# Cyan4973/FiniteStateEntropy

Measured on AMD Instinct MI355X. Metric: MB/s encode+decode per GPU on 32KB probagen blocks; bit-exact vs CPU ref, higher is better.
Workload: dtype u8; 1 GPU; probagen Proba14, 100000 x 32KB blocks per GPU, FSE encode+decode (one-shot calls at the reference's default limits: tableLog 11, decode maxLog 12), bit-exact check; blocks_per_gpu=100000, block_bytes=32768, codec=fse, parity=fse: roundtrip-all-blocks

## Files before the change

### finitestateentropy_amd/csrc/fse_tables.hip

```cpp
#include "internal.h"

#include "wave_glue.h"
#include "ncount_reader.h"
#include "fse_wave_build.h"

DEV void fse_wave_build_ctable(const WaveBuildLds& w, const int nn[4], u32 maxSV, u32 tl, u32* img, u32 lane)
{
    u16* const cumAll = w.cumP;
    *(uint2*)(w.nrm + 4 * lane) = make_uint2(((u32)nn[0] & 0xFFFFu) | ((u32)nn[1] << 16), ((u32)nn[2] & 0xFFFFu) | ((u32)nn[3] << 16));
    __syncthreads();
    const u32 ts = 1u << tl;
    u16* const stateTable = (u16*)(img + 1);
    u32* const tt = img + 1 + (ts >> 1);
    {
        u32 eff[4], laneSum = 0;
#pragma unroll
        for (int i = 0; i < 4; ++i) { eff[i] = nn[i] == -1 ? 1u : (u32)nn[i]; laneSum += eff[i]; }
        u32 total;
        u32 run = wb_scan_excl(laneSum, lane, &total);
#pragma unroll
        for (int i = 0; i < 4; ++i) {
            const u32 s = 4 * lane + i;
            cumAll[s] = (u16)run;
            if (s <= maxSV) {
                if (nn[i] == 0) { tt[2 * s] = 0; tt[2 * s + 1] = ((tl + 1) << 16) - ts; }
                else if (nn[i] == -1 || nn[i] == 1) { tt[2 * s] = run - 1u; tt[2 * s + 1] = (tl << 16) - ts; }
                else {
                    const u32 maxBitsOut = tl - hibit32((u32)nn[i] - 1);
                    tt[2 * s] = run - (u32)nn[i];
                    tt[2 * s + 1] = (maxBitsOut << 16) - ((u32)nn[i] << maxBitsOut);
                }
            }
            run += eff[i];
        }
        if (lane == 0) img[0] = tl | (maxSV << 16);
    }
    __syncthreads();
    wave_spread_rank(w, maxSV, tl, lane, [&](u32 s) { return (u32)cumAll[s]; },
                     [&](u32 u, u32 s, u32 r, u32 first) { (void)s; stateTable[first + r] = (u16)(ts + u); });
}

__global__ __launch_bounds__(64) void k_fse_cprep(FseCPrepArgs a, u32 capTs)
{
    extern __shared__ __attribute__((aligned(16))) u8 wbLds[];
    const size_t b = blockIdx.x;
    const u32 lane = threadIdx.x;
    const size_t n = view_size(a.src, b);
    FseMeta m; m.state = 0; m.hdrSize = 0; m.tableLog = 0; m.maxSV = 0; m.pace = 0;
    const size_t top = a.histResults[b];
    size_t result = 0; bool go = false;
    if (n <= 1) result = 0;
    else if (is_err(top)) result = top;
    else if (top == n) result = 1;
    else if (top == 1 || top < (n >> 7)) result = 0;
    else go = true;
    const WaveBuildLds w = wave_build_carve(wbLds, capTs);
    u32* const hdrImg = w.cnt;
    u32 maxSV = 0, tl = 0;
    int nn[4] = { 0, 0, 0, 0 };
    if (go) {
        maxSV = a.maxSVs[b];
        tl = wg_optimal_tablelog(a.tableLogReq, n, maxSV, 2);
        const uint4 cv = ((const uint4*)(a.counts + b * 256))[lane];
        const u32 c[4] = { cv.x, cv.y, cv.z, cv.w };
        for (u32 i = lane; i < 136; i += 64) hdrImg[i] = 0;
        const size_t e = wg_normalize<64>(nn, c, (u64)n, maxSV, tl, lane);
        if (is_err(e)) { result = e; go = false; }
    }
    __syncthreads();
    if (go) {
        const size_t h = wg_write_ncount<64>(hdrImg, a.dstCapacity, nn, maxSV, tl, lane);
        if (is_err(h)) { result = h; go = false; }
        else m.hdrSize = (u32)h;
    }
    __syncthreads();
    if (!go) { if (lane == 0) { a.meta[b] = m; a.results[b] = result; } return; }
    {   u8* const dst = a.dst + b * a.dstStride;
        const u8* const hb = (const u8*)hdrImg;
        for (u32 i = lane; i < m.hdrSize; i += 64) dst[i] = hb[i];
    }
    int top1 = nn[0] > nn[1] ? nn[0] : nn[1]; top1 = nn[2] > top1 ? nn[2] : top1; top1 = nn[3] > top1 ? nn[3] : top1;
    top1 = wave_max_i32(top1);
    m.state = ((u32)top1 * 64u > (63u << tl) || n < FSE_ENC_WAVE_MIN) ? FSE_ENC_LANE : FSE_ENC_PAR;
    {
        u32 present = (nn[0] != 0) + (nn[1] != 0) + (nn[2] != 0) + (nn[3] != 0);
        present = wg_sum<64>(present);
        const u32 mix = (1u << tl) / (present ? present : 1u);
        m.pace = mix < 64u ? 0u : mix < 128u ? 1u : mix < 256u ? 2u : 3u;
    }
    m.tableLog = tl; m.maxSV = maxSV;
    if (lane == 0) a.meta[b] = m;
    fse_wave_build_ctable(w, nn, maxSV, tl, a.ctables + b * a.ctStrideU32, lane);
}

__global__ __launch_bounds__(64) void k_fse_dparse(FseDPrepArgs a)
{
    const size_t b = (size_t)blockIdx.x * 64 + threadIdx.x;
    const u32 lane = threadIdx.x;
    int cls = -1;
    if (b < a.nBlocks) {
        FseMeta m; m.state = 0; m.hdrSize = 0; m.tableLog = 0; m.maxSV = 0; m.pace = 0; m.pace = 0;
        const u8* const in = view_ptr(a.csrc, b);
        const size_t cSize = view_size(a.csrc, b);
        size_t result = 0;
        bool done = false;
        if (a.rawRle) { const size_t orig = a.origSizes ? a.origSizes[b] : a.uniformOrig; done = cSize == orig || cSize == 1; }
        if (!done) do {
            u32 tl = 0, maxSV = 255;
            s16* const norm = a.norms + b * 256;
            const size_t h = ncount_read<1>(norm, &maxSV, &tl, in, cSize);
            if (is_err(h)) { result = h; break; }
            if (tl > a.maxLog) { result = FERR(tableLog_tooLarge); break; }
            cls = FSE_DCLS_REV11;
            if (tl > FSE_DEC_FAST_MAXLOG) {
                int top = 0;
                for (u32 s = 0; s <= maxSV; ++s) top = norm[s] > top ? norm[s] : top;
                cls = 2 * top > (1 << tl) ? FSE_DCLS_PLAIN : FSE_DCLS_REV12;
            }
            m.state = 1u | ((u32)cls << 2); m.hdrSize = (u32)h; m.tableLog = tl; m.maxSV = maxSV;
        } while (0);
        a.meta[b] = m;
        if (m.state == 0 && !done) a.results[b] = result;
    }
    if (cls >= 0) { const size_t bin = view_size(a.csrc, b) >> FSE_DBIN_LOG; cls = cls * FSE_DBINS + (int)(bin < FSE_DBINS - 1 ? bin : FSE_DBINS - 1); }
    const unsigned long long below = (1ull << lane) - 1ull;
    unsigned long long todo = __ballot(cls >= 0);
    while (todo) {
        const int leader = __builtin_ctzll(todo);
        const int c = __shfl(cls, leader, WAVE);
        const unsigned long long mask = __ballot(cls == c);
        u32 base = 0;
        if ((int)lane == leader) {
            base = atomicAdd(&a.counts[c], (u32)__builtin_popcountll(mask));
            atomicAdd(&a.counts[FSE_DCLS_COUNT + c / FSE_DBINS], (u32)__builtin_popcountll(mask));
        }
        base = (u32)__shfl((int)base, leader, WAVE);
        if (cls == c) a.lists[(size_t)c * a.nBlocks + base + (u32)__builtin_popcountll(mask & below)] = (u32)b;
        todo &= ~mask;
    }
}

__global__ __launch_bounds__(64) void k_fse_dbuild(FseDPrepArgs a, u32 capTs, int firstList, int nLists, u32 ldsCapTs)
{
    extern __shared__ __attribute__((aligned(16))) u8 wbLds[];
    {   u32 total = 0;
        for (int k = firstList / (int)FSE_DBINS; k < (firstList + nLists) / (int)FSE_DBINS; ++k) total += a.counts[FSE_DCLS_COUNT + k];
        if (blockIdx.x >= total) return;
    }
    constexpr int MAXL = 2 * FSE_DBINS;
    static_assert(FSE_DBINS % 4 == 0, "the list lengths are read as 16-byte vectors");
    uint4 cv[MAXL / 4];
#pragma unroll
    for (int i = 0; i < MAXL / 4; ++i) cv[i] = 4 * i < nLists ? ((const uint4*)(a.counts + firstList))[i] : make_uint4(0, 0, 0, 0);
    u32 idx = blockIdx.x;
    int c = firstList + nLists;
    {   u32 before = 0; bool found = false;
#pragma unroll
        for (int i = 0; i < MAXL; ++i) {
            const uint4 v = cv[i >> 2];
            const u32 n = (i & 3) == 0 ? v.x : (i & 3) == 1 ? v.y : (i & 3) == 2 ? v.z : v.w;
            const bool here = !found & (i < nLists) & (idx < before + n);
            c = here ? firstList + i : c; idx = here ? idx - before : idx;
            found |= here;
            before += n;
        }
    }
    if (c == firstList + nLists) return;
    const size_t b = a.lists[(size_t)c * a.nBlocks + idx];
    const u32 lane = threadIdx.x;
    const FseMeta m = a.meta[b];
    if (m.state == 0) return;
    const WaveBuildLds w = wave_build_carve(wbLds, ldsCapTs);
    *(uint2*)(w.nrm + 4 * lane) = *(const uint2*)(a.norms + b * 256 + 4 * lane);
    __syncthreads();
    const u32 tl = m.tableLog, ts = 1u << tl;
    const bool rev = ((m.state >> 2) & 3u) != FSE_DCLS_PLAIN;
    u16* const A = a.atab + b * capTs;
    u8* const S = a.symtab + b * capTs;
    const bool fast = wave_spread_rank(w, m.maxSV, tl, lane, [&](u32 s) { return (u32)(int)w.nrm[s]; }, [&](u32 u, u32 s, u32 r, u32 nrm) {
        const int n = (int)nrm;
        const u32 next = (n > 0 ? (u32)n : 1u) + r;
        const u32 nb = tl - hibit32(next);
        const u32 ns = (next << nb) - ts;
        const u32 x = rev ? __brev(u) >> (32u - tl) : u;
        A[x] = rev ? (u16)(nb | ((__brev(ns) >> (32u - tl)) << 5)) : (u16)((ns & 0xFFFu) | (nb << 12));
        S[x] = (u8)s;
    });
    if (lane == 0) a.meta[b].state = m.state | (fast ? 2u : 0u);
}

__global__ __launch_bounds__(256) void k_fse_export_dtable(FseDPrepArgs a, u32 capTs, u32* dtables, size_t dtStrideU32)
{
    const size_t b = blockIdx.x;
    const FseMeta m = a.meta[b];
    if (m.state == 0) return;
    const u32 tl = m.tableLog, ts = 1u << tl;
    const bool rev = ((m.state >> 2) & 3u) != FSE_DCLS_PLAIN;
    const u16* const A = a.atab + b * capTs;
    const u8* const S = a.symtab + b * capTs;
    u32* const dt = dtables + b * dtStrideU32;
    if (threadIdx.x == 0) dt[0] = tl | ((m.state & 2u) ? 1u << 16 : 0u);
    for (u32 x = threadIdx.x; x < ts; x += blockDim.x) {
        const u32 i = rev ? __brev(x) >> (32u - tl) : x;
        const u32 c = A[i];
        const u32 nb = rev ? (c & 31u) : (c >> 12);
        const u32 ns = rev ? __brev(c >> 5) >> (32u - tl) : (c & 0xFFFu);
        dt[1 + x] = ns | ((u32)S[i] << 16) | (nb << 24);
    }
}
hipError_t launch_fse_export_dtables(const FseDPrepArgs& a, u32* dtables, size_t dtStrideU32, hipStream_t s)
{
    if (a.nBlocks == 0) return hipSuccess;
    hipLaunchKernelGGL(k_fse_export_dtable, dim3((unsigned)a.nBlocks), dim3(256), 0, s, a, 1u << a.maxLog, dtables, dtStrideU32);
    return hipGetLastError();
}

DEV size_t fse_norm_load_checked(int nn[4], const s16* nb, u32 maxSV, u32 tl, u32 maxTl, u32 lane)
{
    if (maxSV > 255u) return FERR(maxSymbolValue_tooLarge);
    if (tl > maxTl) return FERR(tableLog_tooLarge);
    if (tl == 0 || tl == 1 || tl == 3) return FERR(GENERIC);
    u32 cells = 0; bool bad = false;
#pragma unroll
    for (int i = 0; i < 4; ++i) {
        nn[i] = 4 * lane + i <= maxSV ? (int)nb[4 * lane + i] : 0;
        bad |= nn[i] < -1;
        cells += nn[i] == -1 ? 1u : nn[i] > 0 ? (u32)nn[i] : 0u;
    }
    cells = wg_sum<64>(cells);
    return (wg_any<64>(bad, lane) || cells != (1u << tl)) ? FERR(GENERIC) : 0;
}
__global__ __launch_bounds__(64) void k_fse_ctable_from_norm(const s16* norms, size_t normStride, const u32* maxSVs, u32 tl, u32* ctables, size_t ctStrideU32,
                                                            size_t* results, u32 capTs)
{
    extern __shared__ __attribute__((aligned(16))) u8 wbLds[];
    const size_t b = blockIdx.x;
    const u32 lane = threadIdx.x;
    const u32 maxSV = maxSVs[b];
    int nn[4] = { 0, 0, 0, 0 };
    const size_t r = fse_norm_load_checked(nn, norms + b * normStride, maxSV, tl, FSE_MAX_TL, lane);
    if (lane == 0) results[b] = r;
    if (is_err(r)) return;
    fse_wave_build_ctable(wave_build_carve(wbLds, capTs), nn, maxSV, tl, ctables + b * ctStrideU32, lane);
}
hipError_t launch_fse_ctable_from_norm(const s16* norms, size_t normStride, const u32* maxSVs, u32 tl, u32* ctables, size_t ctStrideU32, size_t* results,
                                       size_t nBlocks, hipStream_t s)
{
    if (nBlocks == 0) return hipSuccess;
    const u32 capTs = 1u << (tl >= 1 && tl <= FSE_MAX_TL ? tl : FSE_MAX_TL);
    hipLaunchKernelGGL(k_fse_ctable_from_norm, dim3((unsigned)nBlocks), dim3(64), wave_build_lds_bytes(capTs), s, norms, normStride, maxSVs, tl, ctables, ctStrideU32,
                       results, capTs);
    return hipGetLastError();
}

__global__ __launch_bounds__(64) void k_fse_dmeta_from_norm(FseDPrepArgs a, const s16* norms, size_t normStride, const u32* maxSVs, u32 tl)
{
    const size_t b = blockIdx.x;
    const u32 lane = threadIdx.x;
    const u32 maxSV = maxSVs[b];
    int nn[4] = { 0, 0, 0, 0 };
    const size_t r = fse_norm_load_checked(nn, norms + b * normStride, maxSV, tl, a.maxLog, lane);
    FseMeta m; m.state = 0; m.hdrSize = 0; m.tableLog = tl; m.maxSV = maxSV; m.pace = 0;
    if (!is_err(r)) {
        *(uint2*)(a.norms + b * 256 + 4 * lane) = make_uint2(((u32)nn[0] & 0xFFFFu) | ((u32)nn[1] << 16), ((u32)nn[2] & 0xFFFFu) | ((u32)nn[3] << 16));
        int top = nn[0] > nn[1] ? nn[0] : nn[1]; top = nn[2] > top ? nn[2] : top; top = nn[3] > top ? nn[3] : top;
        top = wave_max_i32(top);
        const u32 cls = tl <= FSE_DEC_FAST_MAXLOG ? (u32)FSE_DCLS_REV11 : 2 * top > (1 << tl) ? (u32)FSE_DCLS_PLAIN : (u32)FSE_DCLS_REV12;
        m.state = 1u | (cls << 2);
        if (lane == 0) {
            const u32 at = atomicAdd(&a.counts[cls * FSE_DBINS], 1u);
            atomicAdd(&a.counts[FSE_DCLS_COUNT + cls], 1u);
            a.lists[(size_t)cls * FSE_DBINS * a.nBlocks + at] = (u32)b;
        }
    }
    if (lane == 0) { a.meta[b] = m; if (is_err(r)) a.results[b] = r; }
}
hipError_t launch_fse_dprep_from_norm(const FseDPrepArgs& a, const s16* norms, size_t normStride, const u32* maxSVs, u32 tl, hipStream_t s)
{
    if (a.nBlocks == 0) return hipSuccess;
    const u32 capTs = 1u << a.maxLog;
    hipError_t e = launch_zero_u32(a.counts, FSE_DCLS_COUNT + FSE_DCLS_KINDS, s);
    if (e != hipSuccess) return e;
    hipLaunchKernelGGL(k_fse_dmeta_from_norm, dim3((unsigned)a.nBlocks), dim3(64), 0, s, a, norms, normStride, maxSVs, tl);
    const u32 capA = a.maxLog < FSE_DEC_FAST_MAXLOG ? capTs : (1u << FSE_DEC_FAST_MAXLOG);
    hipLaunchKernelGGL(k_fse_dbuild, dim3((unsigned)a.nBlocks), dim3(64), wave_build_lds_bytes(capA), s, a, capTs, (int)FSE_DCLS_REV11 * FSE_DBINS, (int)FSE_DBINS, capA);
    if (a.maxLog > FSE_DEC_FAST_MAXLOG)
        hipLaunchKernelGGL(k_fse_dbuild, dim3((unsigned)a.nBlocks), dim3(64), wave_build_lds_bytes(capTs), s, a, capTs, (int)FSE_DCLS_REV12 * FSE_DBINS, 2 * (int)FSE_DBINS, capTs);
    return hipGetLastError();
}

#ifdef FSE_WB_TIMING
extern "C" __attribute__((visibility("default"))) int FSEHIP_debug_wbTiming(unsigned long long* host) { return (int)hipMemcpyFromSymbol(host, HIP_SYMBOL(g_wbTiming), sizeof(g_wbTiming)); }
#endif
__global__ __launch_bounds__(64) void k_fse_glue_normalize(s16* norms, size_t normStride, u32 tlReq, const u32* counts, size_t countStride,
                                                          const size_t* totals, const u32* maxSVs, size_t* results)
{
    const size_t b = blockIdx.x;
    const u32 lane = threadIdx.x;
    const u32 maxSV = maxSVs[b] > 255u ? 255u : maxSVs[b];
    const u32* const cb = counts + b * countStride;
    u32 c[4];
#pragma unroll
    for (int i = 0; i < 4; ++i) c[i] = 4 * lane + i <= maxSV ? cb[4 * lane + i] : 0u;
    int nn[4] = { 0, 0, 0, 0 };
    const u32 tl = tlReq ? tlReq : FSE_DEF_TL;
    const u64 total = (u64)totals[b];
    size_t r = total ? wg_normalize<64>(nn, c, total, maxSV, tl, lane) : FERR(GENERIC);
    if (!is_err(r)) r = tl;
    s16* const nb = norms + b * normStride;
#pragma unroll
    for (int i = 0; i < 4; ++i) if (4 * lane + i <= maxSV && !is_err(r)) nb[4 * lane + i] = (s16)nn[i];
    if (lane == 0) results[b] = r;
}

__global__ __launch_bounds__(64) void k_fse_glue_write_ncount(u8* headers, size_t headerStride, size_t headerCapacity, const s16* norms, size_t normStride,
                                                             const u32* maxSVs, u32 tl, size_t* results)
{
    __shared__ u32 img[136];
    const size_t b = blockIdx.x;
    const u32 lane = threadIdx.x;
    const u32 maxSV = maxSVs[b];
    size_t r;
    if (tl > FSE_MAX_TL) r = FERR(tableLog_tooLarge);
    else if (tl < FSE_MIN_TL || maxSV > 255u) r = FERR(GENERIC);
    else {
        const s16* const nb = norms + b * normStride;
        int nn[4];
#pragma unroll
        for (int i = 0; i < 4; ++i) nn[i] = 4 * lane + i <= maxSV ? (int)nb[4 * lane + i] : 0;
        for (u32 i = lane; i < 136; i += 64) img[i] = 0;
        __syncthreads();
        r = wg_write_ncount<64>(img, headerCapacity, nn, maxSV, tl, lane);
        __syncthreads();
        if (!is_err(r)) {
            u8* const dst = headers + b * headerStride;
            const u8* const hb = (const u8*)img;
            for (u32 i = lane; i < (u32)r; i += 64) dst[i] = hb[i];
        }
    }
    if (lane == 0) results[b] = r;
}

__global__ __launch_bounds__(64) void k_fse_glue_read_ncount(s16* norms, size_t normStride, u32* maxSVs, u32* tableLogs, BlockView headers, size_t nBlocks, size_t* results)
{
    const size_t b = (size_t)blockIdx.x * 64 + threadIdx.x;
    if (b >= nBlocks) return;
    u32 maxSV = maxSVs[b], tl = 0;
    size_t r;
    if ((size_t)maxSV >= normStride) r = FERR(maxSymbolValue_tooLarge);
    else r = ncount_read<1>(norms + b * normStride, &maxSV, &tl, view_ptr(headers, b), view_size(headers, b));
    if (!is_err(r)) { maxSVs[b] = maxSV; tableLogs[b] = tl; }
    results[b] = r;
}

hipError_t launch_fse_glue_normalize(s16* norms, size_t normStride, u32 tl, const u32* counts, size_t countStride, const size_t* totals, const u32* maxSVs,
                                     size_t* results, size_t nBlocks, hipStream_t s)
{
    if (nBlocks == 0) return hipSuccess;
    hipLaunchKernelGGL(k_fse_glue_normalize, dim3((unsigned)nBlocks), dim3(64), 0, s, norms, normStride, tl, counts, countStride, totals, maxSVs, results);
    return hipGetLastError();
}
hipError_t launch_fse_glue_write_ncount(u8* headers, size_t headerStride, size_t headerCapacity, const s16* norms, size_t normStride, const u32* maxSVs, u32 tl,
                                        size_t* results, size_t nBlocks, hipStream_t s)
{
    if (nBlocks == 0) return hipSuccess;
    hipLaunchKernelGGL(k_fse_glue_write_ncount, dim3((unsigned)nBlocks), dim3(64), 0, s, headers, headerStride, headerCapacity, norms, normStride, maxSVs, tl, results);
    return hipGetLastError();
}
hipError_t launch_fse_glue_read_ncount(s16* norms, size_t normStride, u32* maxSVs, u32* tableLogs, const BlockView& headers, size_t* results, size_t nBlocks, hipStream_t s)
{
    if (nBlocks == 0) return hipSuccess;
    hipLaunchKernelGGL(k_fse_glue_read_ncount, dim3((unsigned)((nBlocks + 63) / 64)), dim3(64), 0, s, norms, normStride, maxSVs, tableLogs, headers, nBlocks, results);
    return hipGetLastError();
}

hipError_t launch_fse_cprep(const FseCPrepArgs& a, hipStream_t s)
{
    if (a.nBlocks == 0) return hipSuccess;
    const u32 capTs = 1u << a.maxTl;
    const size_t ldsBytes = wave_build_lds_bytes(capTs);
    probe_before(PK_FSE_CPREP, s);
    hipLaunchKernelGGL(k_fse_cprep, dim3((unsigned)a.nBlocks), dim3(64), ldsBytes, s, a, capTs);
    probe_after(PK_FSE_CPREP, s);
    return hipGetLastError();
}
hipError_t launch_fse_dprep(const FseDPrepArgs& a, hipStream_t s)
{
    if (a.nBlocks == 0) return hipSuccess;
    const u32 capTs = 1u << a.maxLog;
    hipError_t e = launch_zero_u32(a.counts, FSE_DCLS_COUNT + FSE_DCLS_KINDS, s);
    if (e != hipSuccess) return e;
    probe_before(PK_FSE_DPREP, s);
    hipLaunchKernelGGL(k_fse_dparse, dim3((unsigned)((a.nBlocks + 63) / 64)), dim3(64), 0, s, a);
    const u32 capA = a.maxLog < FSE_DEC_FAST_MAXLOG ? capTs : (1u << FSE_DEC_FAST_MAXLOG);
    hipLaunchKernelGGL(k_fse_dbuild, dim3((unsigned)a.nBlocks), dim3(64), wave_build_lds_bytes(capA), s, a, capTs, (int)FSE_DCLS_REV11 * FSE_DBINS, (int)FSE_DBINS, capA);
    if (a.maxLog > FSE_DEC_FAST_MAXLOG)
        hipLaunchKernelGGL(k_fse_dbuild, dim3((unsigned)a.nBlocks), dim3(64), wave_build_lds_bytes(capTs), s, a, capTs, (int)FSE_DCLS_REV12 * FSE_DBINS, 2 * (int)FSE_DBINS, capTs);
    probe_after(PK_FSE_DPREP, s);
    return hipGetLastError();
}
```

### finitestateentropy_amd/csrc/fse_wave_build.h

```cpp
#pragma once
#include "dev_common.h"

#define WB_MAXSYM 256
#ifndef WB_WIN
#define WB_WIN 64u
#endif
#define WB_TSTEP(ts) (((ts) >> 1) + ((ts) >> 3) + 3)

#ifdef FSE_WB_TIMING
__device__ unsigned long long g_wbTiming[4096 * 8];
#define WBT(k) TT[k] = __builtin_readcyclecounter();
#else
#define WBT(k)
#endif
struct WaveBuildLds {
    s16* nrm;
    u16* cumP;
    u8*  symP;
    u8*  symTab;
    u16* marks;
    u32* cnt;
    u16* coarse;
};
__host__ __device__ inline u32 wb_ci(u32 u) { return u + ((u >> 5) << 1); }
__host__ __device__ inline u32 wb_si(u32 u) { return u + ((u >> 5) << 2); }
#ifndef WB_EXTRA_LDS
#define WB_EXTRA_LDS 0u
#endif
__host__ __device__ inline size_t wb_part_a(u32 capTs) { const size_t m = 2 * (size_t)wb_ci(capTs); return m > WB_WIN * 64 ? m : WB_WIN * 64; }
__host__ __device__ inline size_t wb_part_b(u32 capTs) { const size_t t = wb_si(capTs); return t > WB_WIN * 32 ? t : WB_WIN * 32; }
__host__ __device__ inline size_t wave_build_lds_bytes(u32 capTs) { return wb_part_a(capTs) + wb_part_b(capTs) + 512 + 520 + 256 + WB_EXTRA_LDS; }
DEV WaveBuildLds wave_build_carve(u8* base, u32 capTs)
{
    WaveBuildLds w;
    w.cnt = (u32*)base; w.marks = (u16*)base; base += wb_part_a(capTs);
    w.coarse = (u16*)base; w.symTab = base; base += wb_part_b(capTs);
    w.nrm = (s16*)base; base += 512;
    w.cumP = (u16*)base; base += 520;
    w.symP = base;
    return w;
}

DEV u32 wb_bytesum(u32 v) { return __builtin_amdgcn_sad_u8(v, 0u, 0u); }
DEV u32 wb_scan_excl(u32 v, u32 lane, u32* total)
{
#if FSEHIP_DPP_SCANS
    const u32 incl = group_scan_incl<64, ScanAdd>(v, lane);
    *total = group_last<64>(incl, lane);
#else
    u32 incl = v;
#pragma unroll
    for (int off = 1; off < 64; off <<= 1) { const u32 o = (u32)__shfl_up((int)incl, off, WAVE); if ((int)lane >= off) incl += o; }
    *total = (u32)__shfl((int)incl, 63, WAVE);
#endif
    return incl - v;
}

DEV void wb_opaque(u32& v) { asm volatile("" : "+v"(v)); }
#define WB_MAXC ((1u << FSEHIP_FSE_MAX_TABLELOG) >> 6)

template <class Payload, class Emit>
DEV bool wave_spread_rank(const WaveBuildLds& w, u32 maxSV, u32 tl, u32 lane, Payload&& payload, Emit&& emit)
{
#ifdef FSE_WB_TIMING
    unsigned long long TT[8];
#endif
    WBT(0)
    const u32 ts = 1u << tl, mask = ts - 1, step = WB_TSTEP(ts);
    const u32 C = ts >= 64 ? ts >> 6 : 1;
    const bool act = lane * C < ts;
    const u32 m0 = lane * C;
    u16* const marks = w.marks;
    int n[4];
    {   const uint2 raw = *(const uint2*)(w.nrm + 4 * lane);
        n[0] = (s16)(raw.x & 0xFFFFu); n[1] = (s16)(raw.x >> 16); n[2] = (s16)(raw.y & 0xFFFFu); n[3] = (s16)(raw.y >> 16);
    }
    u32 lanePos = 0, laneLow = 0, laneAny = 0; bool big = false;
#pragma unroll
    for (int i = 0; i < 4; ++i) {
        if (4 * lane + i > maxSV) n[i] = 0;
        lanePos += n[i] > 0 ? (u32)n[i] : 0u; laneLow += n[i] == -1; laneAny += n[i] != 0;
        big |= n[i] >= (int)(ts >> 1);
    }
    u32 totals;
    const u32 base3 = wb_scan_excl(lanePos | (laneLow << 13) | (laneAny << 22), lane, &totals);
    u32 posBase = base3 & 0x1FFFu, lowBase = (base3 >> 13) & 0x1FFu, anyBase = base3 >> 22;
    const u32 nLow = (totals >> 13) & 0x1FFu, nAny = totals >> 22;
    const int high = (int)ts - 1 - (int)nLow;
    if (act) { if (C >= 2) for (u32 i = 0; i < C; i += 2) *(u32*)(marks + wb_ci(m0 + i)) = 0; else marks[wb_ci(m0)] = 0; }
    __syncthreads();
    WBT(1)
#pragma unroll
    for (int i = 0; i < 4; ++i) {
        if (n[i] != 0) w.symP[anyBase++] = (u8)(4 * lane + i);
        if (n[i] > 0) { marks[wb_ci(posBase)] = (u16)(4 * lane + i + 1); posBase += (u32)n[i]; }
        else if (n[i] == -1) { w.symTab[wb_si(ts - 1 - lowBase)] = (u8)(4 * lane + i); ++lowBase; }
    }
    u32 nv = 0;
    if (act) { u32 u = (m0 * step) & mask; for (u32 i = 0; i < C; ++i) { nv += (int)u <= high; u = (u + step) & mask; } }
    u32 totalKept;
    const u32 k0 = wb_scan_excl(nv, lane, &totalKept);
    __syncthreads();
    WBT(2)
    u32 localMax = 0;
    for (u32 i = 0; i < nv; i += 8) {
        u32 v[8];
#pragma unroll
        for (u32 j = 0; j < 8; ++j) { const u32 idx = k0 + i + j; v[j] = marks[wb_ci(idx < ts ? idx : ts - 1)]; }
#pragma unroll
        for (u32 j = 0; j < 8; ++j) if (i + j < nv) localMax = v[j] > localMax ? v[j] : localMax;
    }
    u32 run = localMax;
#if FSEHIP_DPP_SCANS
    run = group_scan_incl<64, ScanMax>(run, lane);
    run = dpp_mov<0x138, 0xF, true>(0u, run);
#else
#pragma unroll
    for (int off = 1; off < 64; off <<= 1) { const u32 o = (u32)__shfl_up((int)run, off, WAVE); if ((int)lane >= off) run = o > run ? o : run; }
    run = (u32)__shfl_up((int)run, 1, WAVE);
    if (lane == 0) run = 0;
#endif
    if (act && nv) {
        u32 u = (m0 * step) & mask, k = k0;
        u32 i = 0;
        for (; i + 8 <= C; i += 8) {
            u32 uu[8], v[8]; bool keep[8];
#pragma unroll
            for (u32 j = 0; j < 8; ++j) {
                uu[j] = u; keep[j] = (int)u <= high;
                v[j] = marks[wb_ci(k < ts ? k : ts - 1)];
                k += keep[j]; u = (u + step) & mask;
            }
#pragma unroll
            for (u32 j = 0; j < 8; ++j) if (keep[j]) { run = v[j] > run ? v[j] : run; w.symTab[wb_si(uu[j])] = (u8)(run - 1u); }
        }
        for (; i < C; ++i) {
            if ((int)u <= high) { const u32 v = marks[wb_ci(k)]; ++k; run = v > run ? v : run; w.symTab[wb_si(u)] = (u8)(run - 1u); }
            u = (u + step) & mask;
        }
    }
    __syncthreads();
    WBT(3)

    const u32 nj = C < 8 ? C : 8;
    u32 sym[WB_MAXC / 4], lr[WB_MAXC / 4];
#pragma unroll
    for (u32 q = 0; q < WB_MAXC / 4; ++q) { sym[q] = 0; lr[q] = 0; }
    if (act) {
        if (C >= 8) {
#pragma unroll
            for (u32 g = 0; g < WB_MAXC / 8; ++g)
                if (8 * g < C) {
                    const u32* const syp = (const u32*)(w.symTab + wb_si(m0 + 8 * g));
                    sym[2 * g] = syp[0]; sym[2 * g + 1] = syp[1];
                }
        } else {
#pragma unroll
            for (u32 j = 0; j < 4; ++j) if (j < C) sym[0] |= (u32)w.symTab[wb_si(m0 + j)] << (8 * j);
        }
    }
    const u32 sh8 = 8 * (lane & 3u), grp = lane >> 2;
    const u32 belowMask = (1u << sh8) - 1u;
    const bool single = maxSV < WB_WIN;
    for (u32 base = 0; base <= maxSV; base += WB_WIN) {
        {   const u32 rows = (maxSV + 1 - base) < WB_WIN ? (maxSV + 1 - base) : WB_WIN;
            for (u32 i = 4 * lane; i < rows * 16; i += 256) *(uint4*)(w.cnt + i) = make_uint4(0, 0, 0, 0);
        }
        __syncthreads();
        if (act) {
#pragma unroll
            for (u32 g = 0; g < WB_MAXC / 8; ++g) {
                if (8 * g >= C) break;
                wb_opaque(sym[2 * g]); wb_opaque(sym[2 * g + 1]);
                u32 old[8]; bool in[8];
#pragma unroll
                for (u32 j = 0; j < 8; ++j) {
                    const u32 s = ((sym[2 * g + (j >> 2)] >> (8 * (j & 3))) & 0xFFu) - base;
                    in[j] = j < nj && (single || s < WB_WIN);
                    old[j] = 0;
                    if (in[j]) old[j] = atomicAdd(&w.cnt[s * 16 + grp], 1u << sh8);
                }
#pragma unroll
                for (u32 h = 0; h < 2; ++h) {
                    u32 r = lr[2 * g + h];
#pragma unroll
                    for (u32 k = 0; k < 4; ++k) {
                        const u32 j = 4 * h + k;
                        if (in[j]) r = (r & ~(0xFFu << (8 * k))) | (((old[j] >> sh8) & 0xFFu) << (8 * k));
                    }
                    lr[2 * g + h] = r;
                }
            }
        }
        __syncthreads();
        WBT(4)
        for (u32 j = lane; j < nAny; j += 64) {
            const u32 s = (u32)w.symP[j] - base;
            if (!single && s >= WB_WIN) continue;
            const uint4* const row = (const uint4*)(w.cnt + s * 16);
            const uint4 c0 = row[0], c1 = row[1], c2 = row[2], c3 = row[3];
            u32 r[16];
            u32 acc = 0;
#define WB_ACC(k, v) r[k] = acc; acc += wb_bytesum(v);
            WB_ACC(0, c0.x) WB_ACC(1, c0.y) WB_ACC(2, c0.z) WB_ACC(3, c0.w) WB_ACC(4, c1.x) WB_ACC(5, c1.y) WB_ACC(6, c1.z) WB_ACC(7, c1.w)
            WB_ACC(8, c2.x) WB_ACC(9, c2.y) WB_ACC(10, c2.z) WB_ACC(11, c2.w) WB_ACC(12, c3.x) WB_ACC(13, c3.y) WB_ACC(14, c3.z) WB_ACC(15, c3.w)
#undef WB_ACC
            uint4* const out = (uint4*)(w.coarse + s * 16);
            out[0] = make_uint4(r[0] | (r[1] << 16), r[2] | (r[3] << 16), r[4] | (r[5] << 16), r[6] | (r[7] << 16));
            out[1] = make_uint4(r[8] | (r[9] << 16), r[10] | (r[11] << 16), r[12] | (r[13] << 16), r[14] | (r[15] << 16));
        }
        __syncthreads();
        WBT(5)
        if (act) {
#pragma unroll
            for (u32 g = 0; g < WB_MAXC / 8; ++g) {
                if (8 * g >= C) break;
                wb_opaque(sym[2 * g]); wb_opaque(sym[2 * g + 1]);
                u32 mg = m0 + 8 * g; wb_opaque(mg);
                u32 sf[8], co[8], cn[8], pl[8]; bool in[8];
#pragma unroll
                for (u32 j = 0; j < 8; ++j) {
                    sf[j] = (sym[2 * g + (j >> 2)] >> (8 * (j & 3))) & 0xFFu;
                    const u32 sw = sf[j] - base;
                    in[j] = j < nj && (single || sw < WB_WIN);
                    const u32 row = in[j] ? sw : 0u;
                    co[j] = w.coarse[row * 16 + grp]; cn[j] = w.cnt[row * 16 + grp]; pl[j] = payload(sf[j]);
                }
#pragma unroll
                for (u32 j = 0; j < 8; ++j) {
                    const u32 local = (lr[2 * g + (j >> 2)] >> (8 * (j & 3))) & 0xFFu;
                    if (in[j]) emit(mg + j, sf[j], local + co[j] + wb_bytesum(cn[j] & belowMask), pl[j]);
                }
            }
        }
        __syncthreads();
    }
    WBT(6)
#ifdef FSE_WB_TIMING
    if (lane == 0 && blockIdx.x < 4096) for (int q = 0; q < 6; ++q) g_wbTiming[8 * blockIdx.x + q] = TT[q + 1] - TT[q];
#endif
    return !__any(big);
}
```

### finitestateentropy_amd/csrc/ncount_reader.h

```cpp
#pragma once
#include "dev_common.h"

DEV u32 hw_ld32(const u8* p) { u32 v; __builtin_memcpy(&v, p, 4); return v; }

struct HeaderWindow {
    const u8* base; long at, end; u32 bits; int skip;
    DEV void open(const u8* p, long n) { base = p; at = 0; end = n; skip = 0; bits = hw_ld32(p); }
    DEV bool can_slide() const { return at <= end - 7 || at + (skip >> 3) <= end - 4; }
    DEV void spend_field(int k)
    {
        skip += k;
        if (can_slide()) { at += skip >> 3; skip &= 7; }
        else { skip -= (int)(8 * (end - 4 - at)); at = end - 4; }
        bits = hw_ld32(base + at) >> (skip & 31);
    }
    DEV void spend_in_register(int k) { bits >>= k; skip += k; }
    DEV void end_of_run()
    {
        skip += 2;
        if (can_slide()) { at += skip >> 3; skip &= 7; bits = hw_ld32(base + at) >> skip; }
        else bits >>= 2;
    }
    DEV void spend_repeat16()
    {
        if (at < end - 5) { at += 2; bits = hw_ld32(base + at) >> skip; }
        else { bits >>= 16; skip += 16; }
    }
};

template <int STRIDE>
DEV size_t ncount_parse(s16* norm, u32* maxSVPtr, u32* tlPtr, const u8* in, long n)
{
    const u32 limit = *maxSVPtr;
    for (u32 s = 0; s <= limit; ++s) norm[s * STRIDE] = 0;
    HeaderWindow w; w.open(in, n);
    const u32 tl = (w.bits & 15u) + FSEHIP_FSE_MIN_TABLELOG;
    if (tl > 15u) return FERR(tableLog_tooLarge);
    *tlPtr = tl;
    w.spend_in_register(4);
    int left = (1 << tl) + 1;
    u32 sym = 0;
    bool afterZero = false;
    while (left > 1 && sym <= limit) {
        if (afterZero) {
            u32 to = sym;
            while ((w.bits & 0xFFFFu) == 0xFFFFu) { to += 24; w.spend_repeat16(); }
            while ((w.bits & 3u) == 3u) { to += 3; w.spend_in_register(2); }
            to += w.bits & 3u;
            if (to > limit) return FERR(maxSymbolValue_tooSmall);
            sym = to;
            w.end_of_run();
        }
        const int threshold = 1 << hibit32((u32)left), spare = 2 * threshold - 1 - left;
        const int width = (int)hibit32((u32)left) + 1;
        int v = (int)(w.bits & (u32)(threshold - 1)), used = width - 1;
        if (v >= spare) {
            v = (int)(w.bits & (u32)(2 * threshold - 1));
            if (v >= threshold) v -= spare;
            used = width;
        }
        --v;
        left -= v < 0 ? -v : v;
        norm[sym * STRIDE] = (s16)v;
        ++sym;
        afterZero = v == 0;
        w.spend_field(used);
    }
    if (left != 1 || w.skip > 32) return FERR(corruption_detected);
    *maxSVPtr = sym - 1;
    return (size_t)(w.at + ((w.skip + 7) >> 3));
}

template <int STRIDE>
DEV size_t ncount_read(s16* norm, u32* maxSVPtr, u32* tlPtr, const u8* in, size_t n)
{
    if (n >= 4) return ncount_parse<STRIDE>(norm, maxSVPtr, tlPtr, in, (long)n);
    u8 tmp[4] = { 0, 0, 0, 0 };
    for (size_t i = 0; i < n; ++i) tmp[i] = in[i];
    const size_t r = ncount_parse<STRIDE>(norm, maxSVPtr, tlPtr, tmp, 4);
    if (!is_err(r) && r > n) return FERR(corruption_detected);
    return r;
}
```

Baseline: 204,900 MiB/s of uncompressed data through encode+decode (whole job).

## Stage header bytes in LDS for decode parse and specialize table build by size

The decode-parse kernel now loads each block's first 256 header bytes into LDS with wide vector loads, then parses the normalized counts from LDS instead of issuing scattered unaligned global loads per field. It also zero-fills the norm rows cooperatively with vector stores and scans the norm array 16 bytes at a time when finding the largest count. The table-build kernels are templated on cells per lane (32 or 64), so tableLog-11 tables use smaller register arrays, and the mark array shrinks from u16 to u8 with a trimmed LDS carve. This adds template instantiations and a new tableLog-too-large guard path, and the LDS staging costs extra LDS and a sync per parse block.

```diff
diff --git a/finitestateentropy_amd/csrc/fse_tables.hip b/finitestateentropy_amd/csrc/fse_tables.hip
--- a/finitestateentropy_amd/csrc/fse_tables.hip
+++ b/finitestateentropy_amd/csrc/fse_tables.hip
@@ -4,6 +4,7 @@
 #include "ncount_reader.h"
 #include "fse_wave_build.h"
 
+template <u32 MAXC>
 DEV void fse_wave_build_ctable(const WaveBuildLds& w, const int nn[4], u32 maxSV, u32 tl, u32* img, u32 lane)
 {
     u16* const cumAll = w.cumP;
@@ -36,10 +37,11 @@
         if (lane == 0) img[0] = tl | (maxSV << 16);
     }
     __syncthreads();
-    wave_spread_rank(w, maxSV, tl, lane, [&](u32 s) { return (u32)cumAll[s]; },
+    wave_spread_rank<MAXC>(w, maxSV, tl, lane, [&](u32 s) { return (u32)cumAll[s]; },
                      [&](u32 u, u32 s, u32 r, u32 first) { (void)s; stateTable[first + r] = (u16)(ts + u); });
 }
 
+template <u32 MAXC>
 __global__ __launch_bounds__(64) void k_fse_cprep(FseCPrepArgs a, u32 capTs)
 {
     extern __shared__ __attribute__((aligned(16))) u8 wbLds[];
@@ -54,13 +56,16 @@
     else if (top == n) result = 1;
     else if (top == 1 || top < (n >> 7)) result = 0;
     else go = true;
-    const WaveBuildLds w = wave_build_carve(wbLds, capTs);
+    const WaveBuildLds w = wave_build_carve(wbLds, capTs, true);
     u32* const hdrImg = w.cnt;
     u32 maxSV = 0, tl = 0;
     int nn[4] = { 0, 0, 0, 0 };
     if (go) {
         maxSV = a.maxSVs[b];
         tl = wg_optimal_tablelog(a.tableLogReq, n, maxSV, 2);
+        if ((1u << tl) > 64u * MAXC || (1u << tl) > capTs) { result = FERR(tableLog_tooLarge); go = false; }
+    }
+    if (go) {
         const uint4 cv = ((const uint4*)(a.counts + b * 256))[lane];
         const u32 c[4] = { cv.x, cv.y, cv.z, cv.w };
         for (u32 i = lane; i < 136; i += 64) hdrImg[i] = 0;
@@ -90,31 +95,44 @@
     }
     m.tableLog = tl; m.maxSV = maxSV;
     if (lane == 0) a.meta[b] = m;
-    fse_wave_build_ctable(w, nn, maxSV, tl, a.ctables + b * a.ctStrideU32, lane);
+    fse_wave_build_ctable<MAXC>(w, nn, maxSV, tl, a.ctables + b * a.ctStrideU32, lane);
 }
 
 __global__ __launch_bounds__(64) void k_fse_dparse(FseDPrepArgs a)
 {
-    const size_t b = (size_t)blockIdx.x * 64 + threadIdx.x;
-    const u32 lane = threadIdx.x;
+    __shared__ __attribute__((aligned(16))) u32 stage[NCS_WORDS];
+    const size_t b0 = (size_t)blockIdx.x * 64, b = b0 + threadIdx.x;
+    const u32 lane = threadIdx.x;
+    const bool have = b < a.nBlocks;
+    const u8* const in = have ? view_ptr(a.csrc, b) : nullptr;
+    const size_t cSize = have ? view_size(a.csrc, b) : 0;
+    bool done = false;
+    if (have && a.rawRle) { const size_t orig = a.origSizes ? a.origSizes[b] : a.uniformOrig; done = cSize == orig || cSize == 1; }
+    const u32 staged = ncount_stage(stage, in, cSize, lane, have && !done);
+    {   uint4* const rows = (uint4*)(a.norms + b0 * 256);
+        const u32 nRows = a.nBlocks - b0 < 64 ? (u32)(a.nBlocks - b0) : 64u;
+        for (u32 i = lane; i < nRows * 32u; i += 64) rows[i] = make_uint4(0, 0, 0, 0);
+    }
+    __syncthreads();
     int cls = -1;
-    if (b < a.nBlocks) {
+    if (have) {
         FseMeta m; m.state = 0; m.hdrSize = 0; m.tableLog = 0; m.maxSV = 0; m.pace = 0; m.pace = 0;
-        const u8* const in = view_ptr(a.csrc, b);
-        const size_t cSize = view_size(a.csrc, b);
         size_t result = 0;
-        bool done = false;
-        if (a.rawRle) { const size_t orig = a.origSizes ? a.origSizes[b] : a.uniformOrig; done = cSize == orig || cSize == 1; }
         if (!done) do {
             u32 tl = 0, maxSV = 255;
             s16* const norm = a.norms + b * 256;
-            const size_t h = ncount_read<1>(norm, &maxSV, &tl, in, cSize);
+            const size_t h = ncount_read_staged(norm, &maxSV, &tl, stage + lane, staged, in, cSize);
             if (is_err(h)) { result = h; break; }
             if (tl > a.maxLog) { result = FERR(tableLog_tooLarge); break; }
             cls = FSE_DCLS_REV11;
             if (tl > FSE_DEC_FAST_MAXLOG) {
                 int top = 0;
-                for (u32 s = 0; s <= maxSV; ++s) top = norm[s] > top ? norm[s] : top;
+                for (u32 i = 0; i <= maxSV >> 3; ++i) {
+                    const uint4 v = ((const uint4*)norm)[i];
+                    const u32 q[4] = { v.x, v.y, v.z, v.w };
+#pragma unroll
+                    for (int k = 0; k < 4; ++k) { const int lo = (s16)(q[k] & 0xFFFFu), hi = (s16)(q[k] >> 16); top = lo > top ? lo : top; top = hi > top ? hi : top; }
+                }
                 cls = 2 * top > (1 << tl) ? FSE_DCLS_PLAIN : FSE_DCLS_REV12;
             }
             m.state = 1u | ((u32)cls << 2); m.hdrSize = (u32)h; m.tableLog = tl; m.maxSV = maxSV;
@@ -140,6 +158,7 @@
     }
 }
 
+template <u32 MAXC>
 __global__ __launch_bounds__(64) void k_fse_dbuild(FseDPrepArgs a, u32 capTs, int firstList, int nLists, u32 ldsCapTs)
 {
     extern __shared__ __attribute__((aligned(16))) u8 wbLds[];
@@ -170,14 +189,18 @@
     const u32 lane = threadIdx.x;
     const FseMeta m = a.meta[b];
     if (m.state == 0) return;
-    const WaveBuildLds w = wave_build_carve(wbLds, ldsCapTs);
+    const u32 tl = m.tableLog, ts = 1u << tl;
+    if (ts > ldsCapTs || ts > 64u * MAXC) {
+        if (lane == 0) { a.meta[b].state = 0; a.results[b] = FERR(tableLog_tooLarge); }
+        return;
+    }
+    const WaveBuildLds w = wave_build_carve(wbLds, ldsCapTs, false);
     *(uint2*)(w.nrm + 4 * lane) = *(const uint2*)(a.norms + b * 256 + 4 * lane);
     __syncthreads();
-    const u32 tl = m.tableLog, ts = 1u << tl;
     const bool rev = ((m.state >> 2) & 3u) != FSE_DCLS_PLAIN;
     u16* const A = a.atab + b * capTs;
     u8* const S = a.symtab + b * capTs;
-    const bool fast = wave_spread_rank(w, m.maxSV, tl, lane, [&](u32 s) { return (u32)(int)w.nrm[s]; }, [&](u32 u, u32 s, u32 r, u32 nrm) {
+    const bool fast = wave_spread_rank<MAXC>(w, m.maxSV, tl, lane, [&](u32 s) { return (u32)(int)w.nrm[s]; }, [&](u32 u, u32 s, u32 r, u32 nrm) {
         const int n = (int)nrm;
         const u32 next = (n > 0 ? (u32)n : 1u) + r;
         const u32 nb = tl - hibit32(next);
@@ -230,6 +253,7 @@
     cells = wg_sum<64>(cells);
     return (wg_any<64>(bad, lane) || cells != (1u << tl)) ? FERR(GENERIC) : 0;
 }
+template <u32 MAXC>
 __global__ __launch_bounds__(64) void k_fse_ctable_from_norm(const s16* norms, size_t normStride, const u32* maxSVs, u32 tl, u32* ctables, size_t ctStrideU32,
                                                             size_t* results, u32 capTs)
 {
@@ -238,19 +262,39 @@
     const u32 lane = threadIdx.x;
     const u32 maxSV = maxSVs[b];
     int nn[4] = { 0, 0, 0, 0 };
-    const size_t r = fse_norm_load_checked(nn, norms + b * normStride, maxSV, tl, FSE_MAX_TL, lane);
+    static_assert(MAXC == 32 || MAXC == 64, "64 * MAXC cells = a table of tableLog 11 or 12");
+    const size_t r = fse_norm_load_checked(nn, norms + b * normStride, maxSV, tl, MAXC == 32 ? 11u : FSE_MAX_TL, lane);
     if (lane == 0) results[b] = r;
     if (is_err(r)) return;
-    fse_wave_build_ctable(wave_build_carve(wbLds, capTs), nn, maxSV, tl, ctables + b * ctStrideU32, lane);
+    fse_wave_build_ctable<MAXC>(wave_build_carve(wbLds, capTs, true), nn, maxSV, tl, ctables + b * ctStrideU32, lane);
 }
 hipError_t launch_fse_ctable_from_norm(const s16* norms, size_t normStride, const u32* maxSVs, u32 tl, u32* ctables, size_t ctStrideU32, size_t* results,
                                        size_t nBlocks, hipStream_t s)
 {
     if (nBlocks == 0) return hipSuccess;
     const u32 capTs = 1u << (tl >= 1 && tl <= FSE_MAX_TL ? tl : FSE_MAX_TL);
-    hipLaunchKernelGGL(k_fse_ctable_from_norm, dim3((unsigned)nBlocks), dim3(64), wave_build_lds_bytes(capTs), s, norms, normStride, maxSVs, tl, ctables, ctStrideU32,
-                       results, capTs);
-    return hipGetLastError();
+    if (wb_small(capTs))
+        hipLaunchKernelGGL(k_fse_ctable_from_norm<32>, dim3((unsigned)nBlocks), dim3(64), wave_build_lds_bytes(capTs, true), s, norms, normStride, maxSVs, tl, ctables,
+                           ctStrideU32, results, capTs);
+    else
+        hipLaunchKernelGGL(k_fse_ctable_from_norm<64>, dim3((unsigned)nBlocks), dim3(64), wave_build_lds_bytes(capTs, true), s, norms, normStride, maxSVs, tl, ctables,
+                           ctStrideU32, results, capTs);
+    return hipGetLastError();
+}
+
+static void launch_fse_dbuild_lists(const FseDPrepArgs& a, u32 capTs, int firstList, int nLists, u32 ldsCapTs, hipStream_t s)
+{
+    if (wb_small(ldsCapTs))
+        hipLaunchKernelGGL(k_fse_dbuild<32>, dim3((unsigned)a.nBlocks), dim3(64), wave_build_lds_bytes(ldsCapTs, false), s, a, capTs, firstList, nLists, ldsCapTs);
+    else
+        hipLaunchKernelGGL(k_fse_dbuild<64>, dim3((unsigned)a.nBlocks), dim3(64), wave_build_lds_bytes(ldsCapTs, false), s, a, capTs, firstList, nLists, ldsCapTs);
+}
+static void launch_fse_dbuilds(const FseDPrepArgs& a, hipStream_t s)
+{
+    const u32 capTs = 1u << a.maxLog;
+    const u32 capA = a.maxLog < FSE_DEC_FAST_MAXLOG ? capTs : (1u << FSE_DEC_FAST_MAXLOG);
+    launch_fse_dbuild_lists(a, capTs, (int)FSE_DCLS_REV11 * FSE_DBINS, (int)FSE_DBINS, capA, s);
+    if (a.maxLog > FSE_DEC_FAST_MAXLOG) launch_fse_dbuild_lists(a, capTs, (int)FSE_DCLS_REV12 * FSE_DBINS, 2 * (int)FSE_DBINS, capTs, s);
 }
 
 __global__ __launch_bounds__(64) void k_fse_dmeta_from_norm(FseDPrepArgs a, const s16* norms, size_t normStride, const u32* maxSVs, u32 tl)
@@ -278,14 +322,10 @@
 hipError_t launch_fse_dprep_from_norm(const FseDPrepArgs& a, const s16* norms, size_t normStride, const u32* maxSVs, u32 tl, hipStream_t s)
 {
     if (a.nBlocks == 0) return hipSuccess;
-    const u32 capTs = 1u << a.maxLog;
     hipError_t e = launch_zero_u32(a.counts, FSE_DCLS_COUNT + FSE_DCLS_KINDS, s);
     if (e != hipSuccess) return e;
     hipLaunchKernelGGL(k_fse_dmeta_from_norm, dim3((unsigned)a.nBlocks), dim3(64), 0, s, a, norms, normStride, maxSVs, tl);
-    const u32 capA = a.maxLog < FSE_DEC_FAST_MAXLOG ? capTs : (1u << FSE_DEC_FAST_MAXLOG);
-    hipLaunchKernelGGL(k_fse_dbuild, dim3((unsigned)a.nBlocks), dim3(64), wave_build_lds_bytes(capA), s, a, capTs, (int)FSE_DCLS_REV11 * FSE_DBINS, (int)FSE_DBINS, capA);
-    if (a.maxLog > FSE_DEC_FAST_MAXLOG)
-        hipLaunchKernelGGL(k_fse_dbuild, dim3((unsigned)a.nBlocks), dim3(64), wave_build_lds_bytes(capTs), s, a, capTs, (int)FSE_DCLS_REV12 * FSE_DBINS, 2 * (int)FSE_DBINS, capTs);
+    launch_fse_dbuilds(a, s);
     return hipGetLastError();
 }
 
@@ -378,24 +418,21 @@
 {
     if (a.nBlocks == 0) return hipSuccess;
     const u32 capTs = 1u << a.maxTl;
-    const size_t ldsBytes = wave_build_lds_bytes(capTs);
+    const size_t ldsBytes = wave_build_lds_bytes(capTs, true);
     probe_before(PK_FSE_CPREP, s);
-    hipLaunchKernelGGL(k_fse_cprep, dim3((unsigned)a.nBlocks), dim3(64), ldsBytes, s, a, capTs);
+    if (wb_small(capTs)) hipLaunchKernelGGL(k_fse_cprep<32>, dim3((unsigned)a.nBlocks), dim3(64), ldsBytes, s, a, capTs);
+    else hipLaunchKernelGGL(k_fse_cprep<64>, dim3((unsigned)a.nBlocks), dim3(64), ldsBytes, s, a, capTs);
     probe_after(PK_FSE_CPREP, s);
     return hipGetLastError();
 }
 hipError_t launch_fse_dprep(const FseDPrepArgs& a, hipStream_t s)
 {
     if (a.nBlocks == 0) return hipSuccess;
-    const u32 capTs = 1u << a.maxLog;
     hipError_t e = launch_zero_u32(a.counts, FSE_DCLS_COUNT + FSE_DCLS_KINDS, s);
     if (e != hipSuccess) return e;
     probe_before(PK_FSE_DPREP, s);
     hipLaunchKernelGGL(k_fse_dparse, dim3((unsigned)((a.nBlocks + 63) / 64)), dim3(64), 0, s, a);
-    const u32 capA = a.maxLog < FSE_DEC_FAST_MAXLOG ? capTs : (1u << FSE_DEC_FAST_MAXLOG);
-    hipLaunchKernelGGL(k_fse_dbuild, dim3((unsigned)a.nBlocks), dim3(64), wave_build_lds_bytes(capA), s, a, capTs, (int)FSE_DCLS_REV11 * FSE_DBINS, (int)FSE_DBINS, capA);
-    if (a.maxLog > FSE_DEC_FAST_MAXLOG)
-        hipLaunchKernelGGL(k_fse_dbuild, dim3((unsigned)a.nBlocks), dim3(64), wave_build_lds_bytes(capTs), s, a, capTs, (int)FSE_DCLS_REV12 * FSE_DBINS, 2 * (int)FSE_DBINS, capTs);
+    launch_fse_dbuilds(a, s);
     probe_after(PK_FSE_DPREP, s);
     return hipGetLastError();
 }
diff --git a/finitestateentropy_amd/csrc/fse_wave_build.h b/finitestateentropy_amd/csrc/fse_wave_build.h
--- a/finitestateentropy_amd/csrc/fse_wave_build.h
+++ b/finitestateentropy_amd/csrc/fse_wave_build.h
@@ -18,28 +18,29 @@
     u16* cumP;
     u8*  symP;
     u8*  symTab;
-    u16* marks;
+    u8*  marks;
     u32* cnt;
     u16* coarse;
 };
-__host__ __device__ inline u32 wb_ci(u32 u) { return u + ((u >> 5) << 1); }
 __host__ __device__ inline u32 wb_si(u32 u) { return u + ((u >> 5) << 2); }
 #ifndef WB_EXTRA_LDS
 #define WB_EXTRA_LDS 0u
 #endif
-__host__ __device__ inline size_t wb_part_a(u32 capTs) { const size_t m = 2 * (size_t)wb_ci(capTs); return m > WB_WIN * 64 ? m : WB_WIN * 64; }
-__host__ __device__ inline size_t wb_part_b(u32 capTs) { const size_t t = wb_si(capTs); return t > WB_WIN * 32 ? t : WB_WIN * 32; }
-__host__ __device__ inline size_t wave_build_lds_bytes(u32 capTs) { return wb_part_a(capTs) + wb_part_b(capTs) + 512 + 520 + 256 + WB_EXTRA_LDS; }
-DEV WaveBuildLds wave_build_carve(u8* base, u32 capTs)
+__host__ __device__ inline size_t wb_up16(size_t n) { return (n + 15) & ~(size_t)15; }
+__host__ __device__ inline size_t wb_part_a(u32 capTs) { const size_t m = wb_si(capTs); return wb_up16(m > WB_WIN * 64 ? m : WB_WIN * 64); }
+__host__ __device__ inline size_t wb_part_b(u32 capTs) { const size_t t = wb_si(capTs); return wb_up16(t > WB_WIN * 32 ? t : WB_WIN * 32); }
+__host__ __device__ inline size_t wave_build_lds_bytes(u32 capTs, bool withCum) { return wb_part_a(capTs) + wb_part_b(capTs) + 512 + 256 + (withCum ? 528 : 0) + WB_EXTRA_LDS; }
+DEV WaveBuildLds wave_build_carve(u8* base, u32 capTs, bool withCum)
 {
     WaveBuildLds w;
-    w.cnt = (u32*)base; w.marks = (u16*)base; base += wb_part_a(capTs);
+    w.cnt = (u32*)base; w.marks = base; base += wb_part_a(capTs);
     w.coarse = (u16*)base; w.symTab = base; base += wb_part_b(capTs);
     w.nrm = (s16*)base; base += 512;
-    w.cumP = (u16*)base; base += 520;
-    w.symP = base;
+    w.symP = base; base += 256;
+    w.cumP = withCum ? (u16*)base : nullptr;
     return w;
 }
+__host__ __device__ inline bool wb_small(u32 capTs) { return capTs <= 2048u; }
 
 DEV u32 wb_bytesum(u32 v) { return __builtin_amdgcn_sad_u8(v, 0u, 0u); }
 DEV u32 wb_scan_excl(u32 v, u32 lane, u32* total)
@@ -59,7 +60,7 @@
 DEV void wb_opaque(u32& v) { asm volatile("" : "+v"(v)); }
 #define WB_MAXC ((1u << FSEHIP_FSE_MAX_TABLELOG) >> 6)
 
-template <class Payload, class Emit>
+template <u32 MAXC, class Payload, class Emit>
 DEV bool wave_spread_rank(const WaveBuildLds& w, u32 maxSV, u32 tl, u32 lane, Payload&& payload, Emit&& emit)
 {
 #ifdef FSE_WB_TIMING
@@ -70,7 +71,8 @@
     const u32 C = ts >= 64 ? ts >> 6 : 1;
     const bool act = lane * C < ts;
     const u32 m0 = lane * C;
-    u16* const marks = w.marks;
+    static_assert(MAXC % 8 == 0 && MAXC <= WB_MAXC, "cells per lane: whole groups of eight, at most the largest table's");
+    u8* const marks = w.marks;
     int n[4];
     {   const uint2 raw = *(const uint2*)(w.nrm + 4 * lane);
         n[0] = (s16)(raw.x & 0xFFFFu); n[1] = (s16)(raw.x >> 16); n[2] = (s16)(raw.y & 0xFFFFu); n[3] = (s16)(raw.y >> 16);
@@ -87,13 +89,13 @@
     u32 posBase = base3 & 0x1FFFu, lowBase = (base3 >> 13) & 0x1FFu, anyBase = base3 >> 22;
     const u32 nLow = (totals >> 13) & 0x1FFu, nAny = totals >> 22;
     const int high = (int)ts - 1 - (int)nLow;
-    if (act) { if (C >= 2) for (u32 i = 0; i < C; i += 2) *(u32*)(marks + wb_ci(m0 + i)) = 0; else marks[wb_ci(m0)] = 0; }
+    if (act) { if (C >= 4) for (u32 i = 0; i < C; i += 4) *(u32*)(marks + wb_si(m0 + i)) = 0; else for (u32 i = 0; i < C; ++i) marks[wb_si(m0 + i)] = 0; }
     __syncthreads();
     WBT(1)
 #pragma unroll
     for (int i = 0; i < 4; ++i) {
         if (n[i] != 0) w.symP[anyBase++] = (u8)(4 * lane + i);
-        if (n[i] > 0) { marks[wb_ci(posBase)] = (u16)(4 * lane + i + 1); posBase += (u32)n[i]; }
+        if (n[i] > 0) { marks[wb_si(posBase)] = (u8)(4 * lane + i); posBase += (u32)n[i]; }
         else if (n[i] == -1) { w.symTab[wb_si(ts - 1 - lowBase)] = (u8)(4 * lane + i); ++lowBase; }
     }
     u32 nv = 0;
@@ -106,7 +108,7 @@
     for (u32 i = 0; i < nv; i += 8) {
         u32 v[8];
 #pragma unroll
-        for (u32 j = 0; j < 8; ++j) { const u32 idx = k0 + i + j; v[j] = marks[wb_ci(idx < ts ? idx : ts - 1)]; }
+        for (u32 j = 0; j < 8; ++j) { const u32 idx = k0 + i + j; v[j] = marks[wb_si(idx < ts ? idx : ts - 1)]; }
 #pragma unroll
         for (u32 j = 0; j < 8; ++j) if (i + j < nv) localMax = v[j] > localMax ? v[j] : localMax;
     }
@@ -128,14 +130,14 @@
 #pragma unroll
             for (u32 j = 0; j < 8; ++j) {
                 uu[j] = u; keep[j] = (int)u <= high;
-                v[j] = marks[wb_ci(k < ts ? k : ts - 1)];
+                v[j] = marks[wb_si(k < ts ? k : ts - 1)];
                 k += keep[j]; u = (u + step) & mask;
             }
 #pragma unroll
-            for (u32 j = 0; j < 8; ++j) if (keep[j]) { run = v[j] > run ? v[j] : run; w.symTab[wb_si(uu[j])] = (u8)(run - 1u); }
+            for (u32 j = 0; j < 8; ++j) if (keep[j]) { run = v[j] > run ? v[j] : run; w.symTab[wb_si(uu[j])] = (u8)run; }
         }
         for (; i < C; ++i) {
-            if ((int)u <= high) { const u32 v = marks[wb_ci(k)]; ++k; run = v > run ? v : run; w.symTab[wb_si(u)] = (u8)(run - 1u); }
+            if ((int)u <= high) { const u32 v = marks[wb_si(k)]; ++k; run = v > run ? v : run; w.symTab[wb_si(u)] = (u8)run; }
             u = (u + step) & mask;
         }
     }
@@ -143,13 +145,13 @@
     WBT(3)
 
     const u32 nj = C < 8 ? C : 8;
-    u32 sym[WB_MAXC / 4], lr[WB_MAXC / 4];
-#pragma unroll
-    for (u32 q = 0; q < WB_MAXC / 4; ++q) { sym[q] = 0; lr[q] = 0; }
+    u32 sym[MAXC / 4], lr[MAXC / 4];
+#pragma unroll
+    for (u32 q = 0; q < MAXC / 4; ++q) { sym[q] = 0; lr[q] = 0; }
     if (act) {
         if (C >= 8) {
 #pragma unroll
-            for (u32 g = 0; g < WB_MAXC / 8; ++g)
+            for (u32 g = 0; g < MAXC / 8; ++g)
                 if (8 * g < C) {
                     const u32* const syp = (const u32*)(w.symTab + wb_si(m0 + 8 * g));
                     sym[2 * g] = syp[0]; sym[2 * g + 1] = syp[1];
@@ -169,7 +171,7 @@
         __syncthreads();
         if (act) {
 #pragma unroll
-            for (u32 g = 0; g < WB_MAXC / 8; ++g) {
+            for (u32 g = 0; g < MAXC / 8; ++g) {
                 if (8 * g >= C) break;
                 wb_opaque(sym[2 * g]); wb_opaque(sym[2 * g + 1]);
                 u32 old[8]; bool in[8];
@@ -213,7 +215,7 @@
         WBT(5)
         if (act) {
 #pragma unroll
-            for (u32 g = 0; g < WB_MAXC / 8; ++g) {
+            for (u32 g = 0; g < MAXC / 8; ++g) {
                 if (8 * g >= C) break;
                 wb_opaque(sym[2 * g]); wb_opaque(sym[2 * g + 1]);
                 u32 mg = m0 + 8 * g; wb_opaque(mg);
diff --git a/finitestateentropy_amd/csrc/ncount_reader.h b/finitestateentropy_amd/csrc/ncount_reader.h
--- a/finitestateentropy_amd/csrc/ncount_reader.h
+++ b/finitestateentropy_amd/csrc/ncount_reader.h
@@ -3,37 +3,74 @@
 
 DEV u32 hw_ld32(const u8* p) { u32 v; __builtin_memcpy(&v, p, 4); return v; }
 
+struct GlobalBytes {
+    const u8* base;
+    DEV u32 ld32(long at) const { return hw_ld32(base + at); }
+};
+
+#define NCS_BYTES 256u
+#define NCS_WORDS (NCS_BYTES / 4u * 64u)
+struct StagedBytes {
+    const u32* words; u32 staged; const u8* base;
+    DEV u32 ld32(long at) const
+    {
+        if (at + 4 > (long)staged) return hw_ld32(base + at);
+        const u32 d = (u32)at >> 2, last = (staged >> 2) - 1u;
+        const u32 lo = words[d * 64u], hi = words[(d < last ? d + 1u : last) * 64u];
+        return __builtin_amdgcn_alignbyte(hi, lo, (u32)at & 3u);
+    }
+};
+DEV u32 ncount_stage(u32* stage, const u8* in, size_t n, u32 lane, bool active)
+{
+    constexpr u32 PIECES = NCS_BYTES / 16u;
+    const u32 pieces = !active ? 0u : (n >> 4) < PIECES ? (u32)(n >> 4) : PIECES;
+    uint4 v[PIECES];
+#pragma unroll
+    for (u32 j = 0; j < PIECES; ++j) {
+        v[j] = make_uint4(0, 0, 0, 0);
+        if (j < pieces) __builtin_memcpy(&v[j], in + 16u * j, 16);
+    }
+    if (active && n < 4) for (size_t i = 0; i < n; ++i) v[0].x |= (u32)in[i] << (8 * i);
+#pragma unroll
+    for (u32 j = 0; j < PIECES; ++j) {
+        u32* const q = stage + (4u * j) * 64u + lane;
+        q[0] = v[j].x; q[64] = v[j].y; q[128] = v[j].z; q[192] = v[j].w;
+    }
+    return active && n < 4 ? 4u : 16u * pieces;
+}
+
+template <class Bytes>
 struct HeaderWindow {
-    const u8* base; long at, end; u32 bits; int skip;
-    DEV void open(const u8* p, long n) { base = p; at = 0; end = n; skip = 0; bits = hw_ld32(p); }
+    Bytes src; long at, end; u32 bits; int skip;
+    DEV void open(const Bytes& from, long n) { src = from; at = 0; end = n; skip = 0; bits = src.ld32(0); }
     DEV bool can_slide() const { return at <= end - 7 || at + (skip >> 3) <= end - 4; }
     DEV void spend_field(int k)
     {
         skip += k;
         if (can_slide()) { at += skip >> 3; skip &= 7; }
         else { skip -= (int)(8 * (end - 4 - at)); at = end - 4; }
-        bits = hw_ld32(base + at) >> (skip & 31);
+        bits = src.ld32(at) >> (skip & 31);
     }
     DEV void spend_in_register(int k) { bits >>= k; skip += k; }
     DEV void end_of_run()
     {
         skip += 2;
-        if (can_slide()) { at += skip >> 3; skip &= 7; bits = hw_ld32(base + at) >> skip; }
+        if (can_slide()) { at += skip >> 3; skip &= 7; bits = src.ld32(at) >> skip; }
         else bits >>= 2;
     }
     DEV void spend_repeat16()
     {
-        if (at < end - 5) { at += 2; bits = hw_ld32(base + at) >> skip; }
+        if (at < end - 5) { at += 2; bits = src.ld32(at) >> skip; }
         else { bits >>= 16; skip += 16; }
     }
 };
 
-template <int STRIDE>
-DEV size_t ncount_parse(s16* norm, u32* maxSVPtr, u32* tlPtr, const u8* in, long n)
+template <int STRIDE, bool CLEAR = true, class Bytes>
+DEV size_t ncount_parse(s16* norm, u32* maxSVPtr, u32* tlPtr, const Bytes& in, long n)
 {
     const u32 limit = *maxSVPtr;
-    for (u32 s = 0; s <= limit; ++s) norm[s * STRIDE] = 0;
-    HeaderWindow w; w.open(in, n);
+    if (CLEAR) for (u32 s = 0; s <= limit; ++s) norm[s * STRIDE] = 0;
+    HeaderWindow<Bytes> w; w.open(in, n);
     const u32 tl = (w.bits & 15u) + FSEHIP_FSE_MIN_TABLELOG;
     if (tl > 15u) return FERR(tableLog_tooLarge);
     *tlPtr = tl;
@@ -74,10 +111,16 @@
 template <int STRIDE>
 DEV size_t ncount_read(s16* norm, u32* maxSVPtr, u32* tlPtr, const u8* in, size_t n)
 {
-    if (n >= 4) return ncount_parse<STRIDE>(norm, maxSVPtr, tlPtr, in, (long)n);
+    if (n >= 4) return ncount_parse<STRIDE>(norm, maxSVPtr, tlPtr, GlobalBytes{ in }, (long)n);
     u8 tmp[4] = { 0, 0, 0, 0 };
     for (size_t i = 0; i < n; ++i) tmp[i] = in[i];
-    const size_t r = ncount_parse<STRIDE>(norm, maxSVPtr, tlPtr, tmp, 4);
+    const size_t r = ncount_parse<STRIDE>(norm, maxSVPtr, tlPtr, GlobalBytes{ tmp }, 4);
     if (!is_err(r) && r > n) return FERR(corruption_detected);
     return r;
 }
+DEV size_t ncount_read_staged(s16* norm, u32* maxSVPtr, u32* tlPtr, const u32* words, u32 staged, const u8* in, size_t n)
+{
+    const size_t r = ncount_parse<1, false>(norm, maxSVPtr, tlPtr, StagedBytes{ words, staged, in }, n < 4 ? 4 : (long)n);
+    if (n < 4 && !is_err(r) && r > n) return FERR(corruption_detected);
+    return r;
+}
```

Result: faster. 207,100 MiB/s of uncompressed data through encode+decode (whole job) (median of 6 runs) (+1.1%).
